# sdrobert/pydrobert-speech

Hardware: AMD Instinct MI355X
Metric: frames/s (whole node) + HBM-roofline %, 40-mel fbank 16kHz 25/10ms (higher is better)
Workload: dtype f32

## Files before the change

pydrobert-speech_amd/csrc/pds_internal.h:

```cpp
#pragma once
#include <hip/hip_runtime.h>
#include <stdint.h>

#include <exception>
#include <new>
#include <string>

#include "../../include/pds_amd.h"

namespace pds {

void set_error(const std::string &msg);
int32_t hip_fail(hipError_t err, const char *what);

#define PDS_HIP(call)                                       \
  do {                                                      \
    hipError_t _e = (call);                                 \
    if (_e != hipSuccess) return pds::hip_fail(_e, #call);  \
  } while (0)

struct FastTables {
  int kind = 0;
  int n1 = 0, n2 = 0;
  int rows = 0;
  int num_cus = 0;
  float *d_window = nullptr;
  float *d_twiddle = nullptr;
  float *d_tw_special = nullptr;
  float *d_win_half = nullptr;
  float *d_tw_seed = nullptr;
  float *d_ell_w = nullptr;
  int32_t *d_ell_meta = nullptr;
  int32_t *d_ell_len = nullptr;
  int32_t *d_ell_woff = nullptr;
  int ell_wfloats = 0, ell_slots = 0;
  float *d_seg_w = nullptr;
  int32_t *d_seg_meta = nullptr;
  int seg_rounds = 0, seg_len = 0, seg_wfloats = 0, seg_meta_ints = 0;
  float *d_rs_w = nullptr;
  int32_t *d_rs_meta = nullptr;
  int rs_rounds = 0, rs_len = 0, rs_wfloats = 0;
  float *d_rsn_w = nullptr;
  int32_t *d_rsn_meta = nullptr;
  int rsn_rounds = 0, rsn_len = 0, rsn_wfloats = 0;
  int rs_eslot = -1;
  float *d_ms_w = nullptr;
  int32_t *d_ms_meta = nullptr;
  int ms_rounds = 0, ms_len = 0, ms_wfloats = 0, ms_meta_ints = 0, ms_slots = 0;
  long ms_reads = 0;
  int walk = 0;
  long rs_reads = 0, rs_cost = 0, ell_reads = 0, seg_reads = 0;
  float *d_mf_tab = nullptr;
  int mf_rows = 0;
};

}

struct pds_stft_plan {
  pds_stft_desc d;
  int device = 0;
  int num_bins = 0;
  float *d_window_f32 = nullptr;
  double *d_window_f64 = nullptr;
  int32_t *d_row_ptr = nullptr;
  int32_t *d_col = nullptr;
  float *d_val_f32 = nullptr;
  double *d_val_f64 = nullptr;
  float2 *d_tw_f32 = nullptr;
  double2 *d_tw_f64 = nullptr;
  pds::FastTables fast;
};

namespace pds {
struct SiFftTables {
  int blocks = 0;
  bool big = false;
  float2 *d_spectra = nullptr;
  float2 *d_twiddle = nullptr;
  float2 *d_twiddle2k = nullptr;
  int num_cus = 0;
};
}
// ... 113 lines not shown
```

pydrobert-speech_amd/csrc/stft_fast.hip:

```cpp
#include "stft_wave_launch.h"

namespace pds {

#if PDS_STAMPS
unsigned long long *g_stamp_buf = nullptr;
extern "C" __attribute__((visibility("default"))) void pds_debug_set_stamp_buffer(unsigned long long *d_buf) {
  g_stamp_buf = d_buf;
}
#endif

extern "C" __attribute__((visibility("default"))) int32_t pds_build_experiments(void) { return PDS_EXPERIMENTS ? 1 : 0; }

bool fast_has_f64in(const pds_stft_plan *plan) { return plan->fast.kind && fast_f64in_kind(plan->fast.kind); }

static int fast_geometry_rows(const FastTables &ft, int *minw);

bool fast_has_fused_cmvn(const pds_stft_plan *plan) {
  const FastTables &ft = plan->fast;
  int minw = 0;
  if (!ft.kind || ft.n2 != 16 || (ft.n1 != 32 && ft.n1 != 64) || !fast_geometry_rows(ft, &minw)) return false;
  return ft.walk == 1 || ft.walk == 3 || (ft.walk == 2 && minw <= 2);
}

bool fast_has_fused_deltas(const pds_stft_plan *plan) {
// ... 102 lines not shown
    case 400: n1 = 25; n2 = 16; break;
    case 480: n1 = 30; n2 = 16; break;
    case 640: n1 = 20; n2 = 32; break;
    case 800: n1 = 25; n2 = 32; break;
    case 960: n1 = 30; n2 = 32; break;
    default: return PDS_OK;
  }
  const bool pow2 = (n1 & (n1 - 1)) == 0;
  if (!pow2 && d.frame_length != d.dft_size) return PDS_OK;
  const char *off = std::getenv("PDS_STFT_GENERIC");
  if (off && off[0] == '1') return PDS_OK;
  if (d.frame_length > d.dft_size || d.frame_length <= d.dft_size / 2) return PDS_OK;
  if (d.frame_shift >= (1 << 22)) return PDS_OK;
  if (d.use_log && !((float)d.log_floor >= 1.17549435e-38f)) return PDS_OK;
  if (d.num_filts > 32767) return PDS_OK;
  const int N = d.dft_size, H1 = n1 / 2, cols = (n1 - 1) / 2 + 1;
  std::vector<float> win((size_t)n1 * n2, 0.0f);
  for (int r = 0; r < n2; ++r)
    for (int k = 0; k < n1; ++k) {
      const int idx = n2 * k + r;
      if (idx < d.frame_length) {
        const float w = (float)window[idx];
        win[(size_t)r * n1 + k] = w == 0.0f ? 0x1p-100f : w;
      }
    }
  std::vector<float> tw((size_t)n2 * cols * 2, 0.0f);
  for (int r = 0; r < n2; ++r)
    for (int k1 = 1; k1 < cols; ++k1) {
      const double ang = -2.0 * M_PI * (double)((r * k1) % N) / (double)N;
      const double scale = (!pow2 || PDS_RDFT_DIT) ? 1.0 : (2 * k1 == H1) ? 1.0 : 0.5;
      tw[((size_t)r * cols + k1) * 2 + 0] = (float)(scale * std::cos(ang));
      tw[((size_t)r * cols + k1) * 2 + 1] = (float)(scale * std::sin(ang));
    }
  std::vector<int32_t> order(d.num_filts);
  for (int f = 0; f < d.num_filts; ++f) order[f] = f;
  auto span = [&](int f) {
    return row_ptr[f + 1] > row_ptr[f] ? col[row_ptr[f + 1] - 1] - (col[row_ptr[f]] & ~3) + 1 : 0;
  };
  std::stable_sort(order.begin(), order.end(), [&](int x, int y) { return span(x) > span(y); });
  const int slots = (d.num_filts + n2 - 1) / n2;
  const int pstr = ((N / 2 + 2 + 15) / 32) * 32 + 16;
  std::vector<int32_t> ell_meta((size_t)std::max(slots, 1) * n2, 0), ell_len(std::max(slots, USLOTS), 0),
      ell_woff(std::max(slots, USLOTS), 0);
  std::vector<float> ell_w;
  for (int sl = 0; sl < slots; ++sl) {
    int longest = 8;
    std::vector<int> first(n2, 0);
    for (int j = 0; j < n2 && sl * n2 + j < d.num_filts; ++j) {
      const int f = order[sl * n2 + j];
      if (row_ptr[f + 1] == row_ptr[f]) continue;
      first[j] = col[row_ptr[f]] & ~3;
      longest = std::max(longest, (span(f) + 7) / 8 * 8);
    }
    {
      std::vector<int> lanes;
      for (int j = 0; j < n2 && sl * n2 + j < d.num_filts; ++j)
        if (span(order[sl * n2 + j]) > 0) lanes.push_back(j);
      std::stable_sort(lanes.begin(), lanes.end(), [&](int x, int y) {
        return span(order[sl * n2 + x]) > span(order[sl * n2 + y]);
      });
      std::vector<std::vector<int>> taken(16);
      for (int j : lanes) {
        const int slack = std::min((longest - span(order[sl * n2 + j])) / 4, first[j] / 4);
        int best_shift = 0, best_cost = 1 << 30;
        for (int sh = 0; sh <= slack; ++sh) {
          const int q = first[j] / 4 - sh;
// ... 63 lines not shown
                        : 5 * reads <= 4 * ell_reads || (slots >= 4 && reads < ell_reads);
    };
    const bool want = wanted(best_reads);
    dense_bank = any_reads > 0 && wanted(any_reads);
    dense_reads = any_reads;
    if (best_len && want) {
      const int len = best_len, nslots = best_rounds * 64, wstride = len + 4;
      std::vector<float> seg_w((size_t)nslots * wstride, 0.0f);
      std::vector<int32_t> seg_meta((size_t)nslots + d.num_filts, 0);
      int slot = 0;
      bool ok = true;
      for (int f = 0; f < d.num_filts && ok; ++f) {
        const int count = (span(f) + len - 1) / len;
        seg_meta[(size_t)nslots + f] = slot | (count << 16);
        const int base = count ? col[row_ptr[f]] & ~3 : 0;
        for (int k = 0; k < count; ++k, ++slot) {
          int first = base + k * len;
          if (first + len > pstr) first = (pstr - len) & ~3;
          if (first < 0) ok = false;
          seg_meta[slot] = first;
          for (int q = row_ptr[f]; q < row_ptr[f + 1]; ++q) {
            if (col[q] < base + k * len || col[q] >= base + (k + 1) * len) continue;
            const int t = col[q] - first;
            if (t < 0 || t >= len) ok = false; else seg_w[(size_t)slot * wstride + t] = (float)val[q];
          }
        }
      }
      if (ok) {
        ft.seg_reads = best_reads;
        ft.seg_rounds = best_rounds;
        ft.seg_len = len;
        ft.seg_wfloats = (int)seg_w.size();
        ft.seg_meta_ints = (int)seg_meta.size();
        if (rc == PDS_OK) rc = upload(&ft.d_seg_w, seg_w.data(), seg_w.size());
        if (rc == PDS_OK) rc = upload(&ft.d_seg_meta, seg_meta.data(), seg_meta.size());
      }
    }
  }
  if (n2 == 16 && rc == PDS_OK) {
    RsegTables rs;
    const int area_floats = wave_area_floats(n1, n2);
    if (build_rseg(d.num_filts, row_ptr, col, val, N / 2 + 1, area_floats / 4, 8, rs)) {
      ft.rs_rounds = rs.rounds;
      ft.rs_len = rs.seg_len;
      ft.rs_wfloats = (int)rs.w.size();
      ft.rs_reads = rs.reads_per_lane();
      ft.rs_cost = rs.cost;
      RsegTables rn;
      ft.rs_eslot = -1;
      if (rc == PDS_OK && fast_deltas_kind(N) && build_rseg(d.num_filts, row_ptr, col, val, N / 2 + 1, area_floats / 4, 2, rn, true)) {
        ft.rsn_rounds = rn.rounds;
        ft.rsn_len = rn.seg_len;
        ft.rsn_wfloats = (int)rn.w.size();
        for (size_t at = 0; at < rn.meta.size() && ft.rs_eslot < 0; ++at)
          if ((rn.meta[at] >> 16) == 0) ft.rs_eslot = (int)at;
        rc = upload(&ft.d_rsn_w, rn.w.data(), rn.w.size());
        if (rc == PDS_OK) rc = upload(&ft.d_rsn_meta, rn.meta.data(), rn.meta.size());
      }
      if (rc == PDS_OK) rc = upload(&ft.d_rs_w, rs.w.data(), rs.w.size());
      if (rc == PDS_OK) rc = upload(&ft.d_rs_meta, rs.meta.data(), rs.meta.size());
    }
  }
  if (n2 == 16 && pow2 && rc == PDS_OK && dense_bank) {
    MsegTables ms;
    const int area_floats = wave_area_floats(n1, n2);
    const int max_slots = (area_floats - 4 * pstr) / 16;
    if (build_mseg(d.num_filts, row_ptr, col, val, pstr, max_slots, ms)) {
      ft.ms_rounds = ms.rounds;
      ft.ms_slots = ms.slots;
      ft.ms_len = ms.seg_len;
      ft.ms_wfloats = (int)ms.w.size();
      ft.ms_meta_ints = (int)ms.meta.size();
      ft.ms_reads = ms.reads_per_lane();
      rc = upload(&ft.d_ms_w, ms.w.data(), ms.w.size());
      if (rc == PDS_OK) rc = upload(&ft.d_ms_meta, ms.meta.data(), ms.meta.size());
    }
  }
  {
    const char *force = std::getenv("PDS_STFT_WALK");
    ft.walk = ft.seg_rounds > 0 ? 1 : 0;
    const bool ms_stands_in = ft.walk == 0 && dense_bank && ft.ms_rounds > 0 && N >= PDS_MSEG_MIN_N;
    const long other = ft.walk == 1 ? ft.seg_reads : ms_stands_in ? dense_reads : ft.ell_reads;
    if (ft.rs_rounds > 0 && 10 * ft.rs_reads <= 7 * other) ft.walk = 2;
    if (force && std::strcmp(force, "ell") == 0) ft.walk = 0;
    if (force && std::strcmp(force, "seg") == 0) ft.walk = ft.seg_rounds > 0 ? 1 : 0;
    if (force && std::strcmp(force, "rseg") == 0) ft.walk = ft.rs_rounds > 0 ? 2 : ft.walk;
    if ((ft.walk == 1 || (ft.walk == 0 && ms_stands_in)) && ft.ms_rounds > 0 && N >= PDS_MSEG_MIN_N && !force) ft.walk = 3;
    if (force && std::strcmp(force, "mseg") == 0 && ft.ms_rounds > 0) ft.walk = 3;
    if (std::getenv("PDS_DEBUG_PLAN"))
      std::fprintf(stderr,
                   "pds plan N=%d filters=%d: ell slots %d reads %ld | seg rounds %d len %d reads %ld | rseg rounds %d "
                   "len %d reads %ld cost %ld | mseg rounds %d len %d reads %ld -> walk %d\n",
                   N, d.num_filts, ft.ell_slots, ft.ell_reads, ft.seg_rounds, ft.seg_len, ft.seg_reads, ft.rs_rounds,
                   ft.rs_len, ft.rs_reads, ft.rs_cost, ft.ms_rounds, ft.ms_len, ft.ms_reads, ft.walk);
  }
  if (rc == PDS_OK) rc = upload(&ft.d_ell_w, ell_w.data(), ell_w.size());
  if (rc == PDS_OK) rc = upload(&ft.d_ell_meta, ell_meta.data(), ell_meta.size());
  if (rc == PDS_OK) rc = upload(&ft.d_ell_len, ell_len.data(), ell_len.size());
  if (rc == PDS_OK) rc = upload(&ft.d_ell_woff, ell_woff.data(), ell_woff.size());
  if (rc == PDS_OK) rc = upload(&ft.d_window, win.data(), win.size());
  if (rc == PDS_OK) rc = upload(&ft.d_twiddle, tw.data(), tw.size());
  if (((n1 == 32 || n1 == 64) && n2 == 16) || lean_geometry(n1, n2)) {
    std::vector<float> wh(win), seed((size_t)n2 * 6);
    for (float &v : wh) v *= PDS_RDFT_DIT ? 1.0f : 0.5f;
    const int mult[3] = {1, 4, n1 / 4};
    for (int r = 0; r < n2; ++r)
      for (int j = 0; j < 3; ++j) {
        const double ang = -2.0 * M_PI * (double)((r * mult[j]) % N) / (double)N;
        seed[((size_t)r * 3 + j) * 2 + 0] = (float)std::cos(ang);
        seed[((size_t)r * 3 + j) * 2 + 1] = (float)std::sin(ang);
      }
    if (rc == PDS_OK) rc = upload(&ft.d_win_half, wh.data(), wh.size());
    if (rc == PDS_OK) rc = upload(&ft.d_tw_seed, seed.data(), seed.size());
  }
  std::vector<float> tws((size_t)n2 * 2);
  for (int r = 0; r < n2; ++r) {
    const double ang = -2.0 * M_PI * (double)r / (double)(2 * n2);
    tws[2 * r] = (float)std::cos(ang);
    tws[2 * r + 1] = (float)std::sin(ang);
  }
  if (rc == PDS_OK) rc = upload(&ft.d_tw_special, tws.data(), tws.size());
  {
    const char *front = PDS_EXPERIMENTS ? std::getenv("PDS_STFT_FRONT") : nullptr;
    const int rows = (d.frame_length + n2 - 1) / n2;
    int bucket = 0;
    for (int b : {20, 25, 28, 30, 32})
      if (!bucket && rows <= b) bucket = b;
    MfmaFrontTables mt;
    if (rc == PDS_OK && n1 == 32 && n2 == 16 && bucket && front && std::strcmp(front, "mfma") == 0 &&
        build_mfma_front(n1, bucket, d.frame_length, window, mt)) {
      std::vector<float> image;
      image.reserve(mt.words());
      image.insert(image.end(), mt.win.begin(), mt.win.end());
      for (int32_t v : mt.off) {
        float f;
        std::memcpy(&f, &v, sizeof f);
        image.push_back(f);
      }
      image.insert(image.end(), mt.emask.begin(), mt.emask.end());
      image.insert(image.end(), mt.a_re.begin(), mt.a_re.end());
      image.insert(image.end(), mt.a_im.begin(), mt.a_im.end());
      image.insert(image.end(), mt.tw.begin(), mt.tw.end());
      rc = upload(&ft.d_mf_tab, image.data(), image.size());
      ft.mf_rows = bucket;
    }
  }
  if (rc != PDS_OK) return rc;
  hipDeviceProp_t prop;
  PDS_HIP(hipGetDeviceProperties(&prop, plan->device));
  ft.num_cus = prop.multiProcessorCount;
  ft.n1 = n1;
  ft.n2 = n2;
  ft.rows = (d.frame_length + n2 - 1) / n2;
  ft.kind = d.dft_size;
  return PDS_OK;
}

void fast_tables_destroy(pds_stft_plan *plan) {
  FastTables &ft = plan->fast;
  (void)hipFree(ft.d_window);
  (void)hipFree(ft.d_twiddle);
  (void)hipFree(ft.d_tw_special);
  (void)hipFree(ft.d_win_half);
  (void)hipFree(ft.d_tw_seed);
  (void)hipFree(ft.d_mf_tab);
  (void)hipFree(ft.d_rs_w);
  (void)hipFree(ft.d_ms_w);
  (void)hipFree(ft.d_ms_meta);
  (void)hipFree(ft.d_rsn_w);
  (void)hipFree(ft.d_rsn_meta);
  (void)hipFree(ft.d_rs_meta);
  (void)hipFree(ft.d_seg_w);
  (void)hipFree(ft.d_seg_meta);
  (void)hipFree(ft.d_ell_w);
  (void)hipFree(ft.d_ell_meta);
  (void)hipFree(ft.d_ell_len);
  (void)hipFree(ft.d_ell_woff);
  ft = FastTables();
}

}
```

pydrobert-speech_amd/csrc/stft_switches.h:

```cpp
#pragma once
namespace pds {

#ifndef PDS_PRIO_PACK
#define PDS_PRIO_PACK 0x103212
#endif
#if PDS_PRIO_PACK == 0xffffff
#define PDS_PHASE(i) __builtin_amdgcn_sched_barrier(0)
#else
#define PDS_PHASE(i) do { if (PDS_PRIO_PACK >= 0) __builtin_amdgcn_s_setprio(((PDS_PRIO_PACK) >> (4 * (i))) & 3); } while (0)
#endif
#ifndef PDS_ABLATE
#define PDS_ABLATE 0
#endif
#ifndef PDS_STAMPS
#define PDS_STAMPS 0
#endif
#if PDS_STAMPS
extern unsigned long long *g_stamp_buf;
#define PDS_STAMP(i, drain)                                               \
  do {                                                                    \
    if (PDS_STAMPS == 2) break;                                           \
    __builtin_amdgcn_sched_barrier(0);                                    \
    if (drain) asm volatile("s_waitcnt vmcnt(0)" ::: "memory");           \
    const unsigned long long now_ = __builtin_readcyclecounter();         \
    st_acc[i] += now_ - st_prev;                                          \
    st_prev = now_;                                                       \
    __builtin_amdgcn_sched_barrier(0);                                    \
  } while (0)
#else
#define PDS_STAMP(i, drain) do { } while (0)
#endif
#ifndef PDS_SEG_DEEP_N
#define PDS_SEG_DEEP_N 1024
#endif
#ifndef PDS_ELL_DEEP_N
#define PDS_ELL_DEEP_N 4096
#endif
#ifndef PDS_MSEG_MIN_N
#define PDS_MSEG_MIN_N 1024
#endif
#ifndef PDS_PAIR_SPLIT
#define PDS_PAIR_SPLIT 1
#endif
#ifndef PDS_N4096_MINW
#define PDS_N4096_MINW 2
#endif
#ifndef PDS_FAST_PROLOGUE
#define PDS_FAST_PROLOGUE 1
#endif
#ifndef PDS_MSEG_RED4
#define PDS_MSEG_RED4 1
#endif
#ifndef PDS_FILTER_UNROLL
#define PDS_FILTER_UNROLL 2
#endif
#ifndef PDS_EXPERIMENTS
#define PDS_EXPERIMENTS 0
#endif
#ifndef PDS_RDFT_DIT
#define PDS_RDFT_DIT (!PDS_EXPERIMENTS)
#endif
#ifndef PDS_WINDOW_CONTRACT
#define PDS_WINDOW_CONTRACT 0
#endif
#ifndef PDS_PACKED_LDS
#define PDS_PACKED_LDS 0
#endif
#ifndef PDS_WALK_DPP_FMAC
#define PDS_WALK_DPP_FMAC 1
#endif
#ifndef PDS_PREEMPH_DPP
#define PDS_PREEMPH_DPP 1
#endif
#ifndef PDS_DYN
#define PDS_DYN 0
#endif
#ifndef PDS_PF_TW
#define PDS_PF_TW 1
#endif
#ifndef PDS_LEAN_1024
#define PDS_LEAN_1024 1
// ... 30 lines not shown
```

pydrobert-speech_amd/csrc/stft_wave_kernel.h:

```cpp
#pragma once
#include <algorithm>
#include <atomic>
#include <cmath>
#include <cstdio>
#include <cstdlib>
#include <cstring>
#include <type_traits>
#include <vector>

#include "fft_inlane.h"
#include "mfma_front.h"
#include "rseg_tables.h"
#include "mseg_tables.h"
#include "pds_internal.h"

#include "stft_switches.h"

namespace pds {

__device__ __forceinline__ void keep_alive(float v) { asm volatile("" ::"v"(v)); }

struct FastParams {
  const void *sig;
  const int64_t *offsets, *lengths, *nframes, *row_off;
  void *out;
  int64_t out_stride;
  const float *win_lane;
  const float2 *tw_lane;
  const float2 *tw_special;
  const float *win_half;
  const float2 *tw_seed;
  const float *ell_w;
  const int32_t *ell_meta;
  const int32_t *ell_len;
  const int32_t *ell_woff;
  int ell_wfloats, ell_slots, ell_meta_pad, ell_meta_ints;
  int seg_rounds, seg_len, num_filts;
  int L, S, pad_left, include_energy, use_power, use_log;
  float log_floor, inv_L, preemph;
  double preemph_d;
  int chunks_per_utt, num_utts;
  int waves;
  int area_f;
  unsigned waves_rcp;
  int lds_ticket_off;
  int dyn;
  const float *mf_tab;
  unsigned long long *stamps;
  const int64_t *chunk_prefix;
  double *stat_part;
  int stat_c, stat_cs;
  int lds_stat_off;
  int dl_inner;
  int dl_order;
  int dl_debug;
  int dl_eslot;
  float dl_f1[5], dl_f2[9];
  int step_utts, step_chunks;
};

__device__ __forceinline__ float mul_legacy(float x, float y) {
  float z;
  asm("v_mul_legacy_f32 %0, %1, %2" : "=v"(z) : "v"(x), "v"(y));
  return z;
}

template <int N1>
__device__ __forceinline__ float window_mul(int n1, float x, float w) {
#if PDS_WINDOW_CONTRACT
// ... 46 lines not shown
  const int cols = (n1 - 1) / 2 + 1, groups = 64 / n2, one_pass = groups * cols * (n2 + 2) * 2;
  return (PDS_TWOPASS && n1 == 64 && n2 == 16) ? 2688 : lean_geometry(n1, n2) ? groups * cols * (n2 + 4) : one_pass;
}
constexpr int win_table_stride(int rows) { return ((rows + 3) & ~3) % 8 == 4 ? ((rows + 3) & ~3) : ((rows + 3) & ~3) + 4; }

template <int N1, int N2, int NROWS>
struct WaveGeom {
  static constexpr int N = N1 * N2;
  static constexpr int NREG = (N1 - 1) / 2;
  static constexpr int COLS = NREG + 1;
  static constexpr int CPL = (COLS + N2 - 1) / N2;
  static constexpr bool FULL = COLS % N2 == 0;
  static constexpr bool DIST = N2 >= 16;
  static constexpr int GROUPS = 64 / N2;
  static constexpr int NB = N / 2 + 1;
  static constexpr int RS = N2 + 2;
  static constexpr bool TWOPASS = PDS_TWOPASS && N1 == 64 && N2 == 16;
  static constexpr bool LEAN = lean_geometry(N1, N2);
  static constexpr int RSF = N2 + 4;
  static constexpr int XROWS = TWOPASS ? N2 : COLS;
  static constexpr int EXCH_F2 = wave_area_floats(N1, N2) / 2;
  static_assert(LEAN ? GROUPS * XROWS * RSF <= EXCH_F2 * 2 : GROUPS * XROWS * RS <= EXCH_F2, "the exchange must fit the wave's area");
  static_assert(!LEAN || (CPL == 1 && N2 >= 32), "lean form: one column per lane");
  static constexpr int PSTR = ((NB + 1 + 15) / 32) * 32 + 16;
  static_assert(GROUPS * PSTR <= EXCH_F2 * 2, "P must fit over the exchange area");
  static constexpr int XMIN_F = LEAN ? GROUPS * XROWS * RSF : GROUPS * XROWS * RS * 2;
  static constexpr int GCH = XMIN_F / 64 < NROWS ? XMIN_F / 64 : NROWS;
  static_assert(N % 2 == 0 && CPL >= 1 && N2 <= 64 && (RS * 8) % 16 == 0, "geometry");
  static_assert(inl::is_pow2(N1) ? (FULL || N2 == 2 * COLS) : 600 % N1 == 0,
                "in-lane DFT sizes: 2^k, or a divisor of 600");
  static_assert(NROWS <= N1 && NROWS > 0, "rows");
};

constexpr int USLOTS = 4;

typedef float f32x4 __attribute__((ext_vector_type(4)));

template <int N1, int N2, int NROWS, int MAXWAVES, int MINW, bool ELL_LDS, bool PRE, int SEG = 0, int MF = 0,
          bool RSG = false, typename TIN = float, typename TOUT = float, int DLT = 0, bool STR = false, bool PF = false>
__global__ __launch_bounds__(MAXWAVES * 64, MINW) void stft_wave_kernel(const FastParams p) {
  static_assert(!PF || (DLT == 0 && !STR && MF == 0 && !PRE && std::is_same<TIN, float>::value && (N1 == 32 || N1 == 64) && N2 == 16),
                "prefetch: 16-lane power-of-two geometries, float32 samples, round-robin scheduling");
  constexpr bool STRETCH = DLT > 0 || STR;
  static_assert(!(STR && DLT > 0), "stretch scheduling is part of the fused-deltas launches already");
  static_assert(DLT == 0 || (DLT == 2 && N2 == 16 && RSG && std::is_same<TOUT, float>::value && MF == 0),
                "fused deltas: row-segment walk, float32 features");
  static_assert(MF == 0 || std::is_same<TIN, float>::value, "matrix-pipe front end: float32 samples");
  static_assert(std::is_same<TIN, float>::value || std::is_same<TIN, double>::value || std::is_same<TIN, int16_t>::value, "samples: float32, float64 or int16");
  using G = WaveGeom<N1, N2, NROWS>;
  constexpr int N = G::N, COLS = G::COLS, NREG = G::NREG, RS = G::RS, NB = G::NB, PSTR = G::PSTR;
  constexpr int MSLOTS = 2 * MF + 1;
  static_assert(MF == 0 || (N2 == 16 && N1 == 32 && MF == mfma_front_steps(NROWS)), "matrix-pipe front end: 32 x 16");
  static_assert(MF == 0 || 4 * MSLOTS * 64 <= G::EXCH_F2 * 2, "edge-frame gather reuses the exchange area");
  constexpr int NBP = (NB + 3) / 4 * 4;
  static_assert(!RSG || (G::GROUPS == 4 && ELL_LDS && !SEG && (NBP + 1) * 4 <= G::EXCH_F2 * 2),
                "row-segment walk: four frames per wave, tables in LDS");
  extern __shared__ __attribute__((aligned(16))) float smem[];
  const int lane = threadIdx.x & 63;
  const int wave = __builtin_amdgcn_readfirstlane(threadIdx.x >> 6);
  const int g = lane / N2, r = lane % N2;
  constexpr bool F64S = std::is_same<TIN, double>::value;
  constexpr bool PAIR = F64S && N2 == 16 && MF == 0;
  const int rho = PAIR ? ((r & 7) * 2 + (r >> 3)) : r;
  constexpr int LOADSPAN = PAIR ? (NROWS + 1) / 2 * 32 : NROWS * N2;
  [[maybe_unused]] const unsigned long long st_entry = PDS_STAMPS ? __builtin_readcyclecounter() : 0;
  float *wbase = smem + wave * p.area_f;
  [[maybe_unused]] double *wstat = reinterpret_cast<double *>(smem + p.lds_stat_off) + wave * (2 * p.stat_cs);
// ... 1 lines not shown
  [[maybe_unused]] const bool stats_on = STATS && p.stat_part != nullptr;
  [[maybe_unused]] auto stat_add4 = [&](const int col, const float (&v)[4], const int nf) {
    double t1 = 0.0, t2 = 0.0;
#pragma unroll
    for (int q = 0; q < 4; ++q)
      if (q < nf) {
        const double d = (double)v[q];
        t1 += d;
        t2 = fma(d, d, t2);
      }
    wstat[col] += t1;
    wstat[p.stat_cs + col] += t2;
  };
  float2 *exch = reinterpret_cast<float2 *>(wbase) + g * G::XROWS * RS;
  [[maybe_unused]] float *xf = wbase + g * (G::XROWS * G::RSF);
  float *Pg = wbase + g * PSTR;
  const int nthreads = p.waves * 64;
  float2 *sw_lds = reinterpret_cast<float2 *>(smem + p.waves * p.area_f);
  int *meta_lds = reinterpret_cast<int *>(sw_lds + N2);
  float *ellw_lds = reinterpret_cast<float *>(meta_lds + p.ell_meta_pad);
  constexpr bool TWCHAIN = (PF && PDS_PF_TW == 1) || (PAIR && (N1 == 32 || N1 == 64)) || (PDS_DLT_CHAIN && DLT > 0 && N1 == 32 && N2 == 16) || G::LEAN ||
                           (N1 == 64 && N2 == 16 && (SEG == 2 || PDS_LEAN_1024));
  constexpr bool WINLDS = PF && PDS_PF_WIN == 1;
  constexpr bool WINUSE = G::LEAN || (N1 == 64 && N2 == 16 && (SEG == 2 || PDS_LEAN_1024));
  constexpr int WSTR = win_table_stride(NROWS);
  [[maybe_unused]] float *win_lds = ellw_lds + (ELL_LDS ? p.ell_wfloats : 0);
  if constexpr (WINLDS || WINUSE) {
    const float *wsrc = TWCHAIN ? p.win_half : p.win_lane;
    for (int i = threadIdx.x; i < N2 * WSTR; i += p.waves * 64) {
      const int rr = i / WSTR, k = i - rr * WSTR;
      win_lds[i] = k < NROWS ? wsrc[rr * N1 + k] : 0.0f;
    }
  }
  if (threadIdx.x < N2) sw_lds[threadIdx.x] = p.tw_special[threadIdx.x];
  constexpr bool DYN = PDS_DYN && !STRETCH && !PF;
  [[maybe_unused]] int *ticket_lds = reinterpret_cast<int *>(smem + p.lds_ticket_off);
  if constexpr (DYN) {
    if (threadIdx.x == 0) *ticket_lds = p.waves;
  }
  if constexpr (STR && G::GROUPS == 4 && (SEG != 0 || (RSG && MINW <= 2))) {
    if (p.stat_part) {
      double *z = reinterpret_cast<double *>(smem + p.lds_stat_off);
      for (int i = threadIdx.x; i < p.waves * 2 * p.stat_cs; i += p.waves * 64) z[i] = 0.0;
    }
  }
  if constexpr (RSG) {
    int4 *rec_lds = reinterpret_cast<int4 *>(meta_lds);
    for (int i = threadIdx.x; i < p.seg_rounds * 64; i += nthreads) {
      const int m = p.ell_meta[i], f = (m >> 16) - 1;
      rec_lds[i] = make_int4((m & 0x3fff) * 16, __float_as_int((m & (1 << 14)) ? 1.0f : 0.0f),
                             __float_as_int((m & (1 << 15)) ? 1.0f : 0.0f),
                             f >= 0 ? ((p.include_energy ? 1 : 0) + f) * (int)sizeof(TOUT) : -1);
    }
  } else {
    for (int i = threadIdx.x; i < p.ell_meta_pad; i += nthreads)
      meta_lds[i] = i < p.ell_meta_ints ? p.ell_meta[i] : 0;
  }
#if PDS_FAST_PROLOGUE
  static_assert((G::EXCH_F2 * 2) % 4 == 0, "wave areas are zeroed 16 bytes at a time");
  if constexpr (ELL_LDS) {
    const float4 *src4 = reinterpret_cast<const float4 *>(p.ell_w);
    float4 *dst4 = reinterpret_cast<float4 *>(ellw_lds);
    for (int i = threadIdx.x; i < (p.ell_wfloats >> 2); i += nthreads) dst4[i] = src4[i];
  }
  {
    float4 *z4 = reinterpret_cast<float4 *>(smem);
    for (int i = threadIdx.x; i < p.waves * (p.area_f / 4); i += nthreads) z4[i] = make_float4(0.0f, 0.0f, 0.0f, 0.0f);
  }
#else
  if constexpr (ELL_LDS)
    for (int i = threadIdx.x; i < p.ell_wfloats; i += nthreads) ellw_lds[i] = p.ell_w[i];
  for (int i = threadIdx.x; i < p.waves * p.area_f; i += nthreads) smem[i] = 0.0f;
#endif
  __syncthreads();

  [[maybe_unused]] float win[(MF || WINLDS || WINUSE) ? 1 : NROWS];
  [[maybe_unused]] float twr[(MF || TWCHAIN) ? 1 : COLS], twi[(MF || TWCHAIN) ? 1 : COLS];
  [[maybe_unused]] float sd[6] = {0.0f, 0.0f, 0.0f, 0.0f, 0.0f, 0.0f};
  [[maybe_unused]] float mwin[MSLOTS], mare[MF + 1], maim[MF + 1], mtwr[4], mtwi[4];
  [[maybe_unused]] unsigned moff[MSLOTS];
  if constexpr (MF > 0) {
    const float *tab = p.mf_tab;
#pragma unroll
    for (int sl = 0; sl < MSLOTS; ++sl) {
      mwin[sl] = tab[sl * 64 + lane];
      moff[sl] = (unsigned)reinterpret_cast<const int *>(tab)[(MSLOTS + sl) * 64 + lane] * 4u;
    }
#pragma unroll
    for (int t = 0; t <= MF; ++t) {
      mare[t] = tab[(3 * MSLOTS + t) * 64 + lane];
      maim[t] = tab[(3 * MSLOTS + MF + 1 + t) * 64 + lane];
    }
#pragma unroll
    for (int v = 0; v < 4; ++v) {
      const float2 t = reinterpret_cast<const float2 *>(tab + (3 * MSLOTS + 2 * (MF + 1)) * 64)[v * 64 + lane];
      mtwr[v] = t.x;
      mtwi[v] = t.y;
    }
  } else {
    if constexpr (!WINLDS && !WINUSE) {
      const float *wsrc = TWCHAIN ? p.win_half : p.win_lane;
#pragma unroll
      for (int n1 = 0; n1 < NROWS; ++n1) win[n1] = wsrc[rho * N1 + n1];
    }
    if constexpr (TWCHAIN) {
#pragma unroll
      for (int j = 0; j < 3; ++j) {
        const float2 t = p.tw_seed[rho * 3 + j];
        sd[2 * j] = t.x;
        sd[2 * j + 1] = t.y;
      }
    } else {
#pragma unroll
      for (int k1 = 1; k1 <= NREG; ++k1) {
        const float2 t = p.tw_lane[rho * COLS + k1];
        twr[k1] = t.x;
        twi[k1] = t.y;
      }
    }
  }
  [[maybe_unused]] float pfv[PF ? NROWS : 1];
  [[maybe_unused]] float wl[WINLDS ? NROWS : 1];
  [[maybe_unused]] auto read_window = [&]() {
    if constexpr (WINLDS) {
      const float4 *w4 = reinterpret_cast<const float4 *>(win_lds + rho * WSTR);
#pragma unroll
      for (int j = 0; j < (NROWS + 3) / 4; ++j) {
        const float4 w = w4[j];
        const float wv[4] = {w.x, w.y, w.z, w.w};
#pragma unroll
        for (int u = 0; u < 4; ++u)
          if (4 * j + u < NROWS) wl[4 * j + u] = wv[u];
      }
    }
  };
  read_window();
  [[maybe_unused]] bool pf_ready = false;
  [[maybe_unused]] const int pf_lane = __mul24(g, p.S) + r;
  const int L = p.L, S = p.S;
  const bool use_power = p.use_power != 0;
  const int col0 = p.include_energy ? 1 : 0;

  int b = 0;
  int wg = blockIdx.x;
#ifndef PDS_NO_XCD_MAP
  if ((gridDim.x & 7) == 0) wg = (wg & 7) * (gridDim.x >> 3) + (wg >> 3);
#endif
  int chunk = wg * p.waves + wave;
  if constexpr (!STRETCH) {
    while (chunk >= p.chunks_per_utt && b < p.num_utts) {
      chunk -= p.chunks_per_utt;
      ++b;
    }
  }
  [[maybe_unused]] int rnd = 0, rb = 0, rc = wg * p.waves;
  if constexpr (DYN) {
    while (rc >= p.chunks_per_utt && rb < p.num_utts) {
      rc -= p.chunks_per_utt;
      ++rb;
    }
  }
  [[maybe_unused]] auto take_ticket = [&](const int t) {
    const int jn = (int)__umulhi((unsigned)t, p.waves_rcp), o = t - jn * p.waves;
    while (rnd < jn && rb < p.num_utts) {
      rc += p.step_chunks;
      rb += p.step_utts;
      if (rc >= p.chunks_per_utt) {
        rc -= p.chunks_per_utt;
        ++rb;
// ... 91 lines not shown
        const int l = lane < full ? lane : full - 1;
        float4 val[4];
#pragma unroll
        for (int q = 0; q < 4; ++q) val[q] = *reinterpret_cast<const float4 *>(stage + q * WS + 4 * l);
        if (lane < full) {
#pragma unroll
          for (int q = 0; q < 4; ++q) {
            F4 o = {val[q].x, val[q].y, val[q].z, val[q].w};
            *reinterpret_cast<F4 *>(orow + (int64_t)q * p.out_stride + 4 * l) = o;
          }
        }
      } else {
        for (int l0 = 0; l0 < full; l0 += 64) {
          const int l = l0 + lane;
          if (l < full) {
#pragma unroll 1
            for (int q = 0; q < 4; ++q)
              if (q < fh) {
                const float4 val = *reinterpret_cast<const float4 *>(stage + q * WS + 4 * l);
                F4 o = {val.x, val.y, val.z, val.w};
                *reinterpret_cast<F4 *>(orow + (int64_t)q * p.out_stride + 4 * l) = o;
              }
          }
        }
      }
      if (tail) {
        const int q = tail == 1 ? lane : tail == 2 ? lane >> 1 : (lane * 11) >> 5;
        const int jj = lane - q * tail;
        if (q < fh && q < 4) orow[(int64_t)q * p.out_stride + 4 * full + jj] = stage[q * WS + 4 * full + jj];
      }
    }
    wave_sync();
  };
  [[maybe_unused]] unsigned long long st_acc[8] = {0, 0, 0, 0, 0, 0, 0, 0};
  [[maybe_unused]] unsigned long long st_prev = PDS_STAMPS ? __builtin_readcyclecounter() : 0;
  [[maybe_unused]] const unsigned long long st_loop = st_prev;
  while (STRETCH || b < p.num_utts) {
    if constexpr (STRETCH) {
      if (!piece_open) {
        if (left <= 0) break;
        nfr = (int)load_const(p.nframes + b);
        const int chunks_b = (nfr + G::GROUPS - 1) / G::GROUPS;
        if (e_lo >= chunks_b) {
          ++b;
          e_lo = 0;
          continue;
        }
        n = (int)load_const(p.lengths + b);
        sig_off = load_const(p.offsets + b);
        out_row = load_const(p.row_off + b);
        e_hi = e_lo + left < chunks_b ? e_lo + left : chunks_b;
        c_last = DLT > 0 ? (e_hi < chunks_b ? e_hi : chunks_b - 1) : e_hi - 1;
        chunk = DLT > 0 ? (e_lo > 0 ? e_lo - 1 : 0) : e_lo;
        piece_open = true;
        ran = false;
      }
      if constexpr (STR) {
        if (ran) ++chunk;
        ran = true;
      }
      if (chunk > c_last) {
        if (DLT > 0 && c_last < e_hi) {
          float nx[DR][4];
#pragma unroll
          for (int rd = 0; rd < DR; ++rd)
#pragma unroll
// ... 1156 lines not shown
```

pydrobert-speech_amd/csrc/stft_wave_launch.h:

```cpp
#pragma once
#include "stft_wave_kernel.h"

namespace pds {


constexpr bool fast_f64in_kind(int n) { return n == 256 || n == 512 || n == 1024 || n == 2048; }

constexpr bool fast_deltas_kind(int n) { return n == 512 || n == 1024; }


template <int N1, int N2, int NROWS, int MINW>
int32_t launch_wave(const pds_stft_plan *plan, const BatchArgs &a) {
  using G = WaveGeom<N1, N2, NROWS>;
#ifndef PDS_DLT_MINW
#define PDS_DLT_MINW 3
#endif
  constexpr int DMINW = (N1 == 64 && N2 == 16) ? 2 : MINW > PDS_DLT_MINW ? PDS_DLT_MINW : MINW;
  constexpr int CU_WAVES_STFT = 4 * MINW;
  constexpr int F64_MINW = (N1 == 64 && N2 == 16) ? 2 : MINW, F64_WAVES = 4 * F64_MINW;
  const int CU_WAVES = a.dl_K > 0 ? 4 * DMINW : a.in_f64 ? F64_WAVES : CU_WAVES_STFT;
  const FastTables &ft = plan->fast;
  FastParams p;
  p.sig = a.d_signal;
  p.offsets = a.d_offsets;
  p.lengths = a.d_lengths;
  p.nframes = a.d_nframes;
  p.row_off = a.d_row_off;
  p.out = a.d_out;
  p.out_stride = a.out_stride;
  p.win_lane = ft.d_window;
  p.tw_lane = (const float2 *)ft.d_twiddle;
  p.tw_special = (const float2 *)ft.d_tw_special;
  constexpr bool LEAN_ALL = G::LEAN || (PDS_LEAN_1024 && N1 == 64 && N2 == 16);
  p.win_half = LEAN_ALL ? ft.d_win_half : nullptr;
  p.tw_seed = LEAN_ALL ? (const float2 *)ft.d_tw_seed : nullptr;
  p.ell_w = ft.d_ell_w;
  p.ell_meta = ft.d_ell_meta;
  p.ell_len = ft.d_ell_len;
  p.ell_woff = ft.d_ell_woff;
  p.ell_wfloats = ft.ell_wfloats;
  p.ell_slots = ft.ell_slots;
  p.L = plan->d.frame_length;
  p.S = plan->d.frame_shift;
  p.pad_left = a.pad_left;
  p.include_energy = plan->d.include_energy;
  p.use_power = plan->d.use_power;
  p.use_log = plan->d.use_log;
  p.log_floor = (float)plan->d.log_floor;
  p.inv_L = 1.0f / (float)plan->d.frame_length;
  p.num_utts = a.B;
  const int64_t chunks = (a.max_frames + G::GROUPS - 1) / G::GROUPS;
  if (chunks * a.B > 0x7fffffff || chunks > 0x3fffffff || a.out_stride * G::GROUPS > (a.out_f64 ? 0x0fffffff : 0x1fffffff) ||
      a.max_frames * plan->d.frame_shift > 0x7fffffff) {
    set_error("stft_batch: too many frame chunks in one call");
    return PDS_ERR_INVALID;
  }
  p.chunks_per_utt = (int)chunks;
  const size_t lds_cu = 160 * 1024;
  const size_t per_wave = (size_t)G::EXCH_F2 * 8;
  const int stat_c = a.d_stat_part ? plan->d.num_filts + (plan->d.include_energy ? 1 : 0) : 0;
  const int stat_cs = (stat_c + 3) & ~3;
  const size_t stat_pw = (size_t)2 * stat_cs * 8;
  int shapes[4][2] = {{CU_WAVES / 2, 2}, {CU_WAVES, 1}, {CU_WAVES * 3 / 4, 1}, {CU_WAVES * 5 / 8, 1}};
#ifdef PDS_ONE_WG
  shapes[0][0] = CU_WAVES, shapes[0][1] = 1;
#endif
  if (CU_WAVES % 8 != 0) {
    shapes[0][0] = CU_WAVES, shapes[0][1] = 1;
    shapes[1][0] = CU_WAVES * 2 / 3, shapes[1][1] = 1;
    shapes[2][0] = CU_WAVES / 3, shapes[2][1] = 1;
// ... 20 lines not shown
                     ft.d_win_half && ft.d_tw_seed && !(pf_env && pf_env[0] == '0');
  constexpr int PF_WSTR = ((NROWS + 3) & ~3) % 8 == 4 ? ((NROWS + 3) & ~3) : ((NROWS + 3) & ~3) + 4;
  const size_t pf_extra = (PDS_PF_WIN == 1) ? (size_t)N2 * PF_WSTR * 4 : 0;
  const size_t lean_extra = LEAN_ALL ? (size_t)N2 * win_table_stride(NROWS) * 4 : 0;
  const size_t mseg3_extra = LEAN_ALL ? 0 : (size_t)N2 * win_table_stride(NROWS) * 4;
  constexpr bool MSG = G::GROUPS == 4 && inl::is_pow2(N1);
  constexpr bool SEGOK = G::GROUPS == 4 || (inl::is_pow2(N1) && N2 >= 32);
  for (int cand = (G::GROUPS == 4) ? (dl ? 2 : ft.walk) : (SEGOK && ft.walk == 1 ? 1 : 0); cand >= 0 && !in_lds; --cand) {
    if (cand == 3 && (!MSG || ft.ms_rounds == 0 || pre || a.in_f64 || a.in_i16)) continue;
    if ((cand == 2 && !dl && ft.rs_rounds == 0) || (cand == 1 && (ft.seg_rounds == 0 || pre || a.in_f64 || a.in_i16))) continue;
    const int meta_ints = cand == 3 ? ft.ms_meta_ints : cand == 2 ? (dl ? ft.rsn_rounds : ft.rs_rounds) * 64 : cand == 1 ? ft.seg_meta_ints : ft.ell_slots * N2;
    const int meta_pad = cand == 2 ? meta_ints * 4 : (std::max(meta_ints, USLOTS * N2) + 3) / 4 * 4;
    const size_t fixed = (size_t)N2 * 8 + (size_t)meta_pad * 4 + (cand == 2 && pf_ok ? pf_extra : 0) + lean_extra +
                         (cand == 3 && MSEG3 ? mseg3_extra : 0);
    const size_t table_bytes = (size_t)(cand == 3 ? ft.ms_wfloats : cand == 2 ? (dl ? ft.rsn_wfloats : ft.rs_wfloats) : cand == 1 ? ft.seg_wfloats : ft.ell_wfloats) * 4;
    if (cand == 1 && (size_t)G::GROUPS * G::PSTR * 4 + (size_t)ft.seg_rounds * 64 * 4 * G::GROUPS > per_wave) continue;
    if (cand == 3 && (size_t)G::GROUPS * G::PSTR * 4 + (size_t)ft.ms_slots * 64 > per_wave) continue;
    const size_t area_c = (cand == 3 && MSEG3)
                              ? std::max((size_t)G::XMIN_F * 4, (size_t)G::GROUPS * G::PSTR * 4 + (size_t)ft.ms_slots * 64)
                              : per_wave;
    const int ms_shapes[5][2] = {{12, 1}, {11, 1}, {10, 1}, {9, 1}, {8, 1}};
    const int (*try_shapes)[2] = (cand == 3 && MSEG3) ? ms_shapes : shapes;
    for (int si = 0; si < ((cand == 3 && MSEG3) ? 5 : 4); ++si) {
      const int *shape = try_shapes[si];
      if (shape[0] * (area_c + stat_pw) + fixed + table_bytes + 48 <= lds_cu / shape[1]) {
        waves = shape[0];
        wgs_per_cu = shape[1];
        in_lds = true;
        area_bytes = area_c;
        break;
      }
    }
    p.ell_meta_pad = meta_pad;
    p.ell_meta_ints = meta_ints;
    if (in_lds && cand == 3) {
      p.ell_w = ft.d_ms_w;
      p.ell_meta = ft.d_ms_meta;
      p.ell_wfloats = ft.ms_wfloats;
      p.seg_rounds = ft.ms_rounds;
      p.seg_len = ft.ms_len;
    } else if (in_lds && cand == 1) {
      p.ell_w = ft.d_seg_w;
      p.ell_meta = ft.d_seg_meta;
      p.ell_wfloats = ft.seg_wfloats;
      p.seg_rounds = ft.seg_rounds;
      p.seg_len = ft.seg_len;
    } else if (in_lds && cand == 2) {
      p.ell_w = dl ? ft.d_rsn_w : ft.d_rs_w;
      p.ell_meta = dl ? ft.d_rsn_meta : ft.d_rs_meta;
      p.ell_wfloats = dl ? ft.rsn_wfloats : ft.rs_wfloats;
      p.seg_rounds = dl ? ft.rsn_rounds : ft.rs_rounds;
      p.seg_len = dl ? ft.rsn_len : ft.rs_len;
    }
    if (in_lds) walk = cand;
  }
#ifdef PDS_FORCE_WAVES
  if (in_lds && PDS_FORCE_WAVES <= CU_WAVES / 2) waves = PDS_FORCE_WAVES, wgs_per_cu = 2;
#endif
  const size_t fixed = (size_t)N2 * 8 + (size_t)p.ell_meta_pad * 4 + (walk == 2 && in_lds && pf_ok ? pf_extra : 0) + lean_extra +
                       (walk == 3 && in_lds && MSEG3 ? mseg3_extra : 0);
  const size_t table_bytes = (size_t)p.ell_wfloats * 4;
  if (a.in_i16 && !in_lds) {
    set_error("stft_batch_i16in: not served for this plan (filter table outside LDS)");
    return PDS_ERR_INVALID;
  }
  if (pre && !in_lds) {
    if (a.in_f64 || a.out_f64 || a.dl_K > 0 || a.d_stat_part) {
      set_error("stft_batch: fused pre-emphasis with the filter table outside LDS is served for float32 samples and plain "
                "float32 features only");
      return PDS_ERR_INVALID;
    }
    return launch_stft_generic_f32(plan, a);
  }
  p.preemph = (float)a.preemph;
  p.preemph_d = a.preemph;
  p.waves = waves;
  p.mf_tab = ft.d_mf_tab;
#if PDS_STAMPS
  p.stamps = g_stamp_buf;
#else
  p.stamps = nullptr;
#endif
  p.area_f = (int)(area_bytes / 4);
  size_t smem = waves * area_bytes + fixed + (in_lds ? table_bytes : 0);
  smem = (smem + 15) & ~(size_t)15;
  p.lds_ticket_off = (int)(smem / 4);
  smem += 16;
  p.lds_stat_off = (int)(smem / 4);
  smem += (size_t)waves * stat_pw;
  p.stat_part = nullptr;
  p.stat_c = stat_c;
  p.stat_cs = stat_cs;
  p.waves_rcp = (unsigned)((0x100000000ull + (unsigned)waves - 1) / (unsigned)waves);
  {
// ... 194 lines not shown
```

Measured before the change: 4.032 billion.

## Pack twiddles, filter metadata and weights into one contiguous LDS image per plan

Builds on the host a single contiguous image per walk variant holding the special twiddles, pre-decoded metadata records and filter weights. The kernel prologue fills LDS with a straight 16-byte vectorised copy of that image, issuing the first loads into registers early, instead of several separate loops that also decoded metadata per record. Each wave now zeroes only its own area rather than the whole workgroup zeroing all areas, and the window read moves after the setup. This trims per-block prologue latency, in exchange for more plan memory (duplicate images for the f64-output variant) and stricter consistency checks at launch.

```diff
diff --git a/pydrobert-speech_amd/csrc/pds_internal.h b/pydrobert-speech_amd/csrc/pds_internal.h
--- a/pydrobert-speech_amd/csrc/pds_internal.h
+++ b/pydrobert-speech_amd/csrc/pds_internal.h
@@ -26,28 +26,21 @@
   int num_cus = 0;
   float *d_window = nullptr;
   float *d_twiddle = nullptr;
-  float *d_tw_special = nullptr;
   float *d_win_half = nullptr;
   float *d_tw_seed = nullptr;
   float *d_ell_w = nullptr;
-  int32_t *d_ell_meta = nullptr;
   int32_t *d_ell_len = nullptr;
   int32_t *d_ell_woff = nullptr;
   int ell_wfloats = 0, ell_slots = 0;
-  float *d_seg_w = nullptr;
-  int32_t *d_seg_meta = nullptr;
   int seg_rounds = 0, seg_len = 0, seg_wfloats = 0, seg_meta_ints = 0;
-  float *d_rs_w = nullptr;
-  int32_t *d_rs_meta = nullptr;
   int rs_rounds = 0, rs_len = 0, rs_wfloats = 0;
-  float *d_rsn_w = nullptr;
-  int32_t *d_rsn_meta = nullptr;
   int rsn_rounds = 0, rsn_len = 0, rsn_wfloats = 0;
   int rs_eslot = -1;
-  float *d_ms_w = nullptr;
-  int32_t *d_ms_meta = nullptr;
   int ms_rounds = 0, ms_len = 0, ms_wfloats = 0, ms_meta_ints = 0, ms_slots = 0;
   long ms_reads = 0;
+  static constexpr int kImages = 6;
+  void *d_img[kImages] = {nullptr, nullptr, nullptr, nullptr, nullptr, nullptr};
+  int img_head16[kImages] = {0, 0, 0, 0, 0, 0}, img_all16[kImages] = {0, 0, 0, 0, 0, 0};
   int walk = 0;
   long rs_reads = 0, rs_cost = 0, ell_reads = 0, seg_reads = 0;
   float *d_mf_tab = nullptr;
diff --git a/pydrobert-speech_amd/csrc/plan_image.h b/pydrobert-speech_amd/csrc/plan_image.h
--- /dev/null
+++ b/pydrobert-speech_amd/csrc/plan_image.h
@@ -0,0 +1,54 @@
+#pragma once
+#include <algorithm>
+#include <cstdint>
+#include <cstring>
+#include <vector>
+
+namespace pds {
+
+constexpr int USLOTS = 4;
+
+inline void rseg_decode_record(int32_t m, int include_energy, int feature_bytes, int32_t rec[4]) {
+  const int f = (m >> 16) - 1;
+  const float m1 = (m & (1 << 14)) ? 1.0f : 0.0f, m2 = (m & (1 << 15)) ? 1.0f : 0.0f;
+  rec[0] = (m & 0x3fff) * 16;
+  std::memcpy(&rec[1], &m1, 4);
+  std::memcpy(&rec[2], &m2, 4);
+  rec[3] = f >= 0 ? ((include_energy ? 1 : 0) + f) * feature_bytes : -1;
+}
+
+inline int plan_image_meta_pad(bool rseg, int meta_ints, int n2) {
+  return rseg ? meta_ints * 4 : (std::max(meta_ints, USLOTS * n2) + 3) / 4 * 4;
+}
+
+struct PlanImage {
+  std::vector<uint32_t> words;
+  int head16 = 0;
+  int all16 = 0;
+};
+
+inline bool build_plan_image(int n2, const float *sw, bool rseg, const int32_t *meta, int meta_ints, int include_energy,
+                             int feature_bytes, const float *w, int wfloats, PlanImage &out) {
+  if (n2 <= 0 || (n2 * 2) % 4 != 0 || meta_ints < 0 || wfloats < 0 || wfloats % 4 != 0) return false;
+  const int meta_pad = plan_image_meta_pad(rseg, meta_ints, n2);
+  out.words.assign((size_t)n2 * 2 + meta_pad + wfloats, 0u);
+  uint32_t *at = out.words.data();
+  std::memcpy(at, sw, (size_t)n2 * 8);
+  at += n2 * 2;
+  if (rseg) {
+    for (int i = 0; i < meta_ints; ++i) {
+      int32_t rec[4];
+      rseg_decode_record(meta[i], include_energy, feature_bytes, rec);
+      std::memcpy(at + 4 * (size_t)i, rec, 16);
+    }
+  } else if (meta_ints > 0) {
+    std::memcpy(at, meta, (size_t)meta_ints * 4);
+  }
+  at += meta_pad;
+  if (wfloats > 0) std::memcpy(at, w, (size_t)wfloats * 4);
+  out.head16 = (n2 * 2 + meta_pad) / 4;
+  out.all16 = (int)(out.words.size() / 4);
+  return true;
+}
+
+}
diff --git a/pydrobert-speech_amd/csrc/stft_fast.hip b/pydrobert-speech_amd/csrc/stft_fast.hip
--- a/pydrobert-speech_amd/csrc/stft_fast.hip
+++ b/pydrobert-speech_amd/csrc/stft_fast.hip
@@ -158,6 +158,27 @@
       tw[((size_t)r * cols + k1) * 2 + 0] = (float)(scale * std::cos(ang));
       tw[((size_t)r * cols + k1) * 2 + 1] = (float)(scale * std::sin(ang));
     }
+  std::vector<float> tws((size_t)n2 * 2);
+  for (int r = 0; r < n2; ++r) {
+    const double ang = -2.0 * M_PI * (double)r / (double)(2 * n2);
+    tws[2 * r] = (float)std::cos(ang);
+    tws[2 * r + 1] = (float)std::sin(ang);
+  }
+  auto upload_image = [&](int which, bool rseg, const std::vector<int32_t> &meta, int meta_ints, int feature_bytes,
+                          const std::vector<float> &w) -> int32_t {
+    PlanImage img;
+    if (!build_plan_image(n2, tws.data(), rseg, meta.data(), meta_ints, d.include_energy, feature_bytes, w.data(),
+                          (int)w.size(), img)) {
+      set_error("stft plan: filter table without an LDS image");
+      return PDS_ERR_INVALID;
+    }
+    ft.img_head16[which] = img.head16;
+    ft.img_all16[which] = img.all16;
+    uint32_t *d_words = nullptr;
+    const int32_t rc_img = upload(&d_words, img.words.data(), img.words.size());
+    ft.d_img[which] = d_words;
+    return rc_img;
+  };
   std::vector<int32_t> order(d.num_filts);
   for (int f = 0; f < d.num_filts; ++f) order[f] = f;
   auto span = [&](int f) {
@@ -287,8 +308,7 @@
         ft.seg_len = len;
         ft.seg_wfloats = (int)seg_w.size();
         ft.seg_meta_ints = (int)seg_meta.size();
-        if (rc == PDS_OK) rc = upload(&ft.d_seg_w, seg_w.data(), seg_w.size());
-        if (rc == PDS_OK) rc = upload(&ft.d_seg_meta, seg_meta.data(), seg_meta.size());
+        if (rc == PDS_OK) rc = upload_image(1, false, seg_meta, (int)seg_meta.size(), 4, seg_w);
       }
     }
   }
@@ -309,11 +329,10 @@
         ft.rsn_wfloats = (int)rn.w.size();
         for (size_t at = 0; at < rn.meta.size() && ft.rs_eslot < 0; ++at)
           if ((rn.meta[at] >> 16) == 0) ft.rs_eslot = (int)at;
-        rc = upload(&ft.d_rsn_w, rn.w.data(), rn.w.size());
-        if (rc == PDS_OK) rc = upload(&ft.d_rsn_meta, rn.meta.data(), rn.meta.size());
-      }
-      if (rc == PDS_OK) rc = upload(&ft.d_rs_w, rs.w.data(), rs.w.size());
-      if (rc == PDS_OK) rc = upload(&ft.d_rs_meta, rs.meta.data(), rs.meta.size());
+        if (rc == PDS_OK) rc = upload_image(4, true, rn.meta, (int)rn.meta.size(), 4, rn.w);
+      }
+      if (rc == PDS_OK) rc = upload_image(2, true, rs.meta, (int)rs.meta.size(), 4, rs.w);
+      if (rc == PDS_OK) rc = upload_image(5, true, rs.meta, (int)rs.meta.size(), 8, rs.w);
     }
   }
   if (n2 == 16 && pow2 && rc == PDS_OK && dense_bank) {
@@ -327,8 +346,7 @@
       ft.ms_wfloats = (int)ms.w.size();
       ft.ms_meta_ints = (int)ms.meta.size();
       ft.ms_reads = ms.reads_per_lane();
-      rc = upload(&ft.d_ms_w, ms.w.data(), ms.w.size());
-      if (rc == PDS_OK) rc = upload(&ft.d_ms_meta, ms.meta.data(), ms.meta.size());
+      if (rc == PDS_OK) rc = upload_image(3, false, ms.meta, (int)ms.meta.size(), 4, ms.w);
     }
   }
   {
@@ -350,7 +368,7 @@
                    ft.rs_len, ft.rs_reads, ft.rs_cost, ft.ms_rounds, ft.ms_len, ft.ms_reads, ft.walk);
   }
   if (rc == PDS_OK) rc = upload(&ft.d_ell_w, ell_w.data(), ell_w.size());
-  if (rc == PDS_OK) rc = upload(&ft.d_ell_meta, ell_meta.data(), ell_meta.size());
+  if (rc == PDS_OK) rc = upload_image(0, false, ell_meta, slots * n2, 4, ell_w);
   if (rc == PDS_OK) rc = upload(&ft.d_ell_len, ell_len.data(), ell_len.size());
   if (rc == PDS_OK) rc = upload(&ft.d_ell_woff, ell_woff.data(), ell_woff.size());
   if (rc == PDS_OK) rc = upload(&ft.d_window, win.data(), win.size());
@@ -368,13 +386,6 @@
     if (rc == PDS_OK) rc = upload(&ft.d_win_half, wh.data(), wh.size());
     if (rc == PDS_OK) rc = upload(&ft.d_tw_seed, seed.data(), seed.size());
   }
-  std::vector<float> tws((size_t)n2 * 2);
-  for (int r = 0; r < n2; ++r) {
-    const double ang = -2.0 * M_PI * (double)r / (double)(2 * n2);
-    tws[2 * r] = (float)std::cos(ang);
-    tws[2 * r + 1] = (float)std::sin(ang);
-  }
-  if (rc == PDS_OK) rc = upload(&ft.d_tw_special, tws.data(), tws.size());
   {
     const char *front = PDS_EXPERIMENTS ? std::getenv("PDS_STFT_FRONT") : nullptr;
     const int rows = (d.frame_length + n2 - 1) / n2;
@@ -415,22 +426,13 @@
   FastTables &ft = plan->fast;
   (void)hipFree(ft.d_window);
   (void)hipFree(ft.d_twiddle);
-  (void)hipFree(ft.d_tw_special);
   (void)hipFree(ft.d_win_half);
   (void)hipFree(ft.d_tw_seed);
   (void)hipFree(ft.d_mf_tab);
-  (void)hipFree(ft.d_rs_w);
-  (void)hipFree(ft.d_ms_w);
-  (void)hipFree(ft.d_ms_meta);
-  (void)hipFree(ft.d_rsn_w);
-  (void)hipFree(ft.d_rsn_meta);
-  (void)hipFree(ft.d_rs_meta);
-  (void)hipFree(ft.d_seg_w);
-  (void)hipFree(ft.d_seg_meta);
   (void)hipFree(ft.d_ell_w);
-  (void)hipFree(ft.d_ell_meta);
   (void)hipFree(ft.d_ell_len);
   (void)hipFree(ft.d_ell_woff);
+  for (void *img : ft.d_img) (void)hipFree(img);
   ft = FastTables();
 }
 
diff --git a/pydrobert-speech_amd/csrc/stft_switches.h b/pydrobert-speech_amd/csrc/stft_switches.h
--- a/pydrobert-speech_amd/csrc/stft_switches.h
+++ b/pydrobert-speech_amd/csrc/stft_switches.h
@@ -45,8 +45,8 @@
 #ifndef PDS_N4096_MINW
 #define PDS_N4096_MINW 2
 #endif
-#ifndef PDS_FAST_PROLOGUE
-#define PDS_FAST_PROLOGUE 1
+#ifndef PDS_STARTUP_BATCH
+#define PDS_STARTUP_BATCH 0
 #endif
 #ifndef PDS_MSEG_RED4
 #define PDS_MSEG_RED4 1
diff --git a/pydrobert-speech_amd/csrc/stft_wave_kernel.h b/pydrobert-speech_amd/csrc/stft_wave_kernel.h
--- a/pydrobert-speech_amd/csrc/stft_wave_kernel.h
+++ b/pydrobert-speech_amd/csrc/stft_wave_kernel.h
@@ -12,6 +12,7 @@
 #include "mfma_front.h"
 #include "rseg_tables.h"
 #include "mseg_tables.h"
+#include "plan_image.h"
 #include "pds_internal.h"
 
 #include "stft_switches.h"
@@ -27,14 +28,14 @@
   int64_t out_stride;
   const float *win_lane;
   const float2 *tw_lane;
-  const float2 *tw_special;
   const float *win_half;
   const float2 *tw_seed;
   const float *ell_w;
-  const int32_t *ell_meta;
   const int32_t *ell_len;
   const int32_t *ell_woff;
-  int ell_wfloats, ell_slots, ell_meta_pad, ell_meta_ints;
+  int ell_wfloats, ell_slots, ell_meta_pad;
+  const void *lds_img;
+  int lds_img16;
   int seg_rounds, seg_len, num_filts;
   int L, S, pad_left, include_energy, use_power, use_log;
   float log_floor, inv_L, preemph;
@@ -147,7 +148,6 @@
   static_assert(NROWS <= N1 && NROWS > 0, "rows");
 };
 
-constexpr int USLOTS = 4;
 
 typedef float f32x4 __attribute__((ext_vector_type(4)));
 
@@ -215,7 +215,6 @@
       win_lds[i] = k < NROWS ? wsrc[rr * N1 + k] : 0.0f;
     }
   }
-  if (threadIdx.x < N2) sw_lds[threadIdx.x] = p.tw_special[threadIdx.x];
   constexpr bool DYN = PDS_DYN && !STRETCH && !PF;
   [[maybe_unused]] int *ticket_lds = reinterpret_cast<int *>(smem + p.lds_ticket_off);
   if constexpr (DYN) {
@@ -227,35 +226,32 @@
       for (int i = threadIdx.x; i < p.waves * 2 * p.stat_cs; i += p.waves * 64) z[i] = 0.0;
     }
   }
-  if constexpr (RSG) {
-    int4 *rec_lds = reinterpret_cast<int4 *>(meta_lds);
-    for (int i = threadIdx.x; i < p.seg_rounds * 64; i += nthreads) {
-      const int m = p.ell_meta[i], f = (m >> 16) - 1;
-      rec_lds[i] = make_int4((m & 0x3fff) * 16, __float_as_int((m & (1 << 14)) ? 1.0f : 0.0f),
-                             __float_as_int((m & (1 << 15)) ? 1.0f : 0.0f),
-                             f >= 0 ? ((p.include_energy ? 1 : 0) + f) * (int)sizeof(TOUT) : -1);
-    }
-  } else {
-    for (int i = threadIdx.x; i < p.ell_meta_pad; i += nthreads)
-      meta_lds[i] = i < p.ell_meta_ints ? p.ell_meta[i] : 0;
+  static_assert((G::EXCH_F2 * 2) % 4 == 0, "wave areas are zeroed 16 bytes at a time");
+  constexpr int IMG_U = (N1 == 64 && N2 == 16) ? 4 : 2;
+  const char *img = static_cast<const char *>(p.lds_img);
+  char *tab = reinterpret_cast<char *>(sw_lds);
+  const unsigned img_bytes = (unsigned)p.lds_img16 * 16u, img_step = (unsigned)nthreads * 16u;
+  float4 imgv[IMG_U];
+  inl::static_for<0, IMG_U>([&](auto uu) {
+    constexpr int u = decltype(uu)::value;
+    const unsigned at = threadIdx.x * 16u + u * img_step;
+    imgv[u] = at < img_bytes ? *reinterpret_cast<const float4 *>(img + at) : make_float4(0.0f, 0.0f, 0.0f, 0.0f);
+  });
+  {
+    float4 *z4 = reinterpret_cast<float4 *>(wbase);
+    for (int i = lane; i < (p.area_f >> 2); i += 64) z4[i] = make_float4(0.0f, 0.0f, 0.0f, 0.0f);
   }
-#if PDS_FAST_PROLOGUE
-  static_assert((G::EXCH_F2 * 2) % 4 == 0, "wave areas are zeroed 16 bytes at a time");
-  if constexpr (ELL_LDS) {
-    const float4 *src4 = reinterpret_cast<const float4 *>(p.ell_w);
-    float4 *dst4 = reinterpret_cast<float4 *>(ellw_lds);
-    for (int i = threadIdx.x; i < (p.ell_wfloats >> 2); i += nthreads) dst4[i] = src4[i];
-  }
-  {
-    float4 *z4 = reinterpret_cast<float4 *>(smem);
-    for (int i = threadIdx.x; i < p.waves * (p.area_f / 4); i += nthreads) z4[i] = make_float4(0.0f, 0.0f, 0.0f, 0.0f);
-  }
-#else
-  if constexpr (ELL_LDS)
-    for (int i = threadIdx.x; i < p.ell_wfloats; i += nthreads) ellw_lds[i] = p.ell_w[i];
-  for (int i = threadIdx.x; i < p.waves * p.area_f; i += nthreads) smem[i] = 0.0f;
-#endif
-  __syncthreads();
+  auto set_up_lds = [&]() {
+    inl::static_for<0, IMG_U>([&](auto uu) {
+      constexpr int u = decltype(uu)::value;
+      const unsigned at = threadIdx.x * 16u + u * img_step;
+      if (at < img_bytes) *reinterpret_cast<float4 *>(tab + at) = imgv[u];
+    });
+    for (unsigned at = threadIdx.x * 16u + IMG_U * img_step; at < img_bytes; at += img_step)
+      *reinterpret_cast<float4 *>(tab + at) = *reinterpret_cast<const float4 *>(img + at);
+    __syncthreads();
+  };
+  if constexpr (!PDS_STARTUP_BATCH) set_up_lds();
 
   [[maybe_unused]] float win[(MF || WINLDS || WINUSE) ? 1 : NROWS];
   [[maybe_unused]] float twr[(MF || TWCHAIN) ? 1 : COLS], twi[(MF || TWCHAIN) ? 1 : COLS];
@@ -317,7 +313,6 @@
       }
     }
   };
-  read_window();
   [[maybe_unused]] bool pf_ready = false;
   [[maybe_unused]] const int pf_lane = __mul24(g, p.S) + r;
   const int L = p.L, S = p.S;
@@ -475,6 +470,8 @@
     }
     wave_sync();
   };
+  if constexpr (PDS_STARTUP_BATCH) set_up_lds();
+  read_window();
   [[maybe_unused]] unsigned long long st_acc[8] = {0, 0, 0, 0, 0, 0, 0, 0};
   [[maybe_unused]] unsigned long long st_prev = PDS_STAMPS ? __builtin_readcyclecounter() : 0;
   [[maybe_unused]] const unsigned long long st_loop = st_prev;
diff --git a/pydrobert-speech_amd/csrc/stft_wave_launch.h b/pydrobert-speech_amd/csrc/stft_wave_launch.h
--- a/pydrobert-speech_amd/csrc/stft_wave_launch.h
+++ b/pydrobert-speech_amd/csrc/stft_wave_launch.h
@@ -30,12 +30,10 @@
   p.out_stride = a.out_stride;
   p.win_lane = ft.d_window;
   p.tw_lane = (const float2 *)ft.d_twiddle;
-  p.tw_special = (const float2 *)ft.d_tw_special;
   constexpr bool LEAN_ALL = G::LEAN || (PDS_LEAN_1024 && N1 == 64 && N2 == 16);
   p.win_half = LEAN_ALL ? ft.d_win_half : nullptr;
   p.tw_seed = LEAN_ALL ? (const float2 *)ft.d_tw_seed : nullptr;
   p.ell_w = ft.d_ell_w;
-  p.ell_meta = ft.d_ell_meta;
   p.ell_len = ft.d_ell_len;
   p.ell_woff = ft.d_ell_woff;
   p.ell_wfloats = ft.ell_wfloats;
@@ -122,22 +120,15 @@
       }
     }
     p.ell_meta_pad = meta_pad;
-    p.ell_meta_ints = meta_ints;
     if (in_lds && cand == 3) {
-      p.ell_w = ft.d_ms_w;
-      p.ell_meta = ft.d_ms_meta;
       p.ell_wfloats = ft.ms_wfloats;
       p.seg_rounds = ft.ms_rounds;
       p.seg_len = ft.ms_len;
     } else if (in_lds && cand == 1) {
-      p.ell_w = ft.d_seg_w;
-      p.ell_meta = ft.d_seg_meta;
       p.ell_wfloats = ft.seg_wfloats;
       p.seg_rounds = ft.seg_rounds;
       p.seg_len = ft.seg_len;
     } else if (in_lds && cand == 2) {
-      p.ell_w = dl ? ft.d_rsn_w : ft.d_rs_w;
-      p.ell_meta = dl ? ft.d_rsn_meta : ft.d_rs_meta;
       p.ell_wfloats = dl ? ft.rsn_wfloats : ft.rs_wfloats;
       p.seg_rounds = dl ? ft.rsn_rounds : ft.rs_rounds;
       p.seg_len = dl ? ft.rsn_len : ft.rs_len;
@@ -150,6 +141,16 @@
   const size_t fixed = (size_t)N2 * 8 + (size_t)p.ell_meta_pad * 4 + (walk == 2 && in_lds && pf_ok ? pf_extra : 0) + lean_extra +
                        (walk == 3 && in_lds && MSEG3 ? mseg3_extra : 0);
   const size_t table_bytes = (size_t)p.ell_wfloats * 4;
+  {
+    const int which = walk == 2 ? (dl ? 4 : a.out_f64 ? 5 : 2) : walk;
+    p.lds_img = ft.d_img[which];
+    p.lds_img16 = in_lds ? ft.img_all16[which] : ft.img_head16[which];
+    if (!p.lds_img || (size_t)ft.img_head16[which] * 16 != (size_t)N2 * 8 + (size_t)p.ell_meta_pad * 4 ||
+        (size_t)ft.img_all16[which] * 16 != (size_t)N2 * 8 + (size_t)p.ell_meta_pad * 4 + table_bytes) {
+      set_error("stft_batch: the plan's LDS image does not match the launch");
+      return PDS_ERR_INVALID;
+    }
+  }
   if (a.in_i16 && !in_lds) {
     set_error("stft_batch_i16in: not served for this plan (filter table outside LDS)");
     return PDS_ERR_INVALID;
```

After: 4.046 billion (median of 6 runs). About the same (+0.4%).
